# jgsimard/RustRobotics

Hardware: AMD Instinct MI355X
Metric: GN iterations/s (higher is better)
Workload: dtype f64; 1 GPU; intel (1728 poses / 4830 edges / dim 5184), Gauss-Newton, one graph on one GPU; solver=GaussNewton, parallelism=single

## Files before the change

### rustrobotics_amd/csrc/kernels.hip.h

```cpp
#pragma once
#include <hip/hip_runtime.h>

#include <cstdint>
#include <type_traits>

#ifndef RRPGO_CHAIN_PRIO
#define RRPGO_CHAIN_PRIO 3
#endif

namespace rrpgo {

constexpr unsigned X_PENDING_WORD = 0x7ff8deadu;

template <typename T> struct VecT;
template <> struct VecT<float> { using V4 = float4; using V2 = float2; };
template <> struct VecT<double> { using V4 = double4; using V2 = double2; };

#ifndef RRPGO_LIN_GROUP
#define RRPGO_LIN_GROUP 8
#endif
constexpr int LIN_GROUP = RRPGO_LIN_GROUP;
constexpr int LIN_THREADS = 256;
constexpr int UPD_THREADS = 256;

// ... 1424 lines not shown
__device__ __forceinline__ void diag16_factor_invert_full(T *P, int M, int k0, int *err, T *wscr) {
  const int lane = threadIdx.x & 63, ll = lane & 31, q = lane & 15;
  const bool rowlane = ll < 16;
  const T *src = rowlane ? P + k0 * M + k0 + q : wscr + 16 * 17 + q;
  const int sstride = rowlane ? M : 16;
  T x[16];
#pragma unroll
  for (int c = 0; c < 16; c++) x[c] = src[c * sstride];
  const bool bad = chol16_dpp2<T>(x);
  if (bad && lane == 0) atomicOr(err, DEVERR_NOT_SPD);
  T *dst = rowlane ? P + k0 * M + k0 + q : wscr + q * 17;
  const int dstride = rowlane ? M : 1;
#pragma unroll
  for (int c = 0; c < 16; c++) dst[c * dstride] = x[c];
}
template <typename T>
__device__ __forceinline__ void diag16_factor_invert_part(T *P, int M, int k0, int nb, int *err, T *wscr) {
  const int lane = threadIdx.x & 63, ll = lane & 31, q = lane & 15;
  const bool rowlane = ll < 16;
  const bool prow = rowlane && q < nb;
  T *ident = wscr + 16 * 17;
  const T *src = prow ? P + k0 * M + k0 + q : ident + q;
  const int sstride = prow ? M : 16;
  T x[16];
#pragma unroll
  for (int c = 0; c < 16; c++) {
    const T *pc = (prow && c >= nb) ? ident + 1 : src + c * sstride;
    x[c] = *pc;
  }
  const bool bad = chol16_dpp2<T>(x, nb);
  if (bad && lane == 0) atomicOr(err, DEVERR_NOT_SPD);
  T *dump = wscr + 16;
  T *dst = prow ? P + k0 * M + k0 + q : rowlane ? dump : wscr + q * 17;
  const int dstride = prow ? M : rowlane ? 0 : 1;
#pragma unroll
  for (int c = 0; c < 16; c++) {
    T *pc = (prow && c >= nb) ? dump : dst + c * dstride;
    *pc = x[c];
  }
}
template <typename T> __device__ __forceinline__ void copy_w16(const T *wscr, T *wout) {
  const int lane = threadIdx.x & 63;
#pragma unroll
  for (int u = 0; u < 4; u++) {
    const int e = lane + 64 * u;
    wout[e] = wscr[(e & 15) * 17 + (e >> 4)];
  }
}
template <typename T> __device__ __forceinline__ void init_w16_identity(T *wscr, int tid, int nthreads) {
  for (int t = tid; t < 256; t += nthreads) wscr[16 * 17 + t] = (t >> 4) == (t & 15) ? (T)1 : (T)0;
}

struct NoUAddr { __device__ float *operator()(int, int) const { return nullptr; } };
template <typename T, int THREADS, bool FAST = false, typename UAddr = NoUAddr>
__device__ __forceinline__ void panel_factor(T *P, int M, int nc, int *err, T *wscr , T *wout,
                             unsigned long long *acc = nullptr, int nu = 0, UAddr uaddr = UAddr(), bool defer_u = false) {
  using MM = Mfma16<T>;
  constexpr int NB = 16;
  constexpr int NW = THREADS / 64;
  const int tid = threadIdx.x;
  const int wave = wave_index(), lane = tid & 63, li = lane & 15, lk = lane >> 4;
  RRPGO_ACC_DECL();
  int pend_k0 = -1;
  auto rest_update = [&](int pk0, int first_wave, int nwaves) {
    const int js = pk0 + NB;
    const int nj = (nc - js + 15) >> 4, ni = (M - js + 15) >> 4;
    int total = 0;
    for (int jb = 1; jb < nj; jb++) total += max(ni - jb, 0);
    const int nt = (nu + 15) >> 4;
    const int utotal = defer_u ? 0 : nt * (nt + 1) / 2;
    for (int t = wave - first_wave; t < total + utotal; t += nwaves) {
      if (t < total) {
        int jb = 1, rem = t;
        while (rem >= ni - jb) { rem -= ni - jb; jb++; }
        const int ib = jb + rem;
        tile_rank_update<T>(P, M, js + 16 * ib, js + 16 * jb, M, nc, pk0, pk0 + NB,
                            [&](int i, int j) { return P + j * M + i; });
      } else {
        if constexpr (!std::is_same<UAddr, NoUAddr>::value) {
          int jb = 0, rem = t - total;
          while (rem >= nt - jb) { rem -= nt - jb; jb++; }
          const int ib = jb + rem;
          tile_rank_update<T>(P + nc, M, 16 * ib, 16 * jb, nu, nu, pk0, pk0 + NB, uaddr);
        }
      }
    }
  };
  for (int k0 = 0; k0 < nc; k0 += NB) {
    const int nb = min(NB, nc - k0);
    RRPGO_ACC_BEGIN();
    constexpr bool fast = FAST;
    auto diag = [&] {
      static_assert(FAST, "the general diagonal-block form (fronts factored in place in global memory by this routine) was retired in r05");
      if (nb == NB) diag16_factor_invert_full<T>(P, M, k0, err, wscr);
      else diag16_factor_invert_part<T>(P, M, k0, nb, err, wscr);
    };
    if (NW == 1) {
      if (pend_k0 >= 0) rest_update(pend_k0, 0, 1);
      diag();
    } else if (wave == 0) {
      diag();
    } else if (pend_k0 >= 0) {
      rest_update(pend_k0, 1, NW - 1);
    }
    pend_k0 = -1;
    __syncthreads();
    RRPGO_ACC_END(acc, 7);
    RRPGO_ACC_BEGIN();
    {
      const int r0 = k0 + nb;
      const int ntiles = (M - r0 + 15) >> 4;
      T wa[4];
#pragma unroll
      for (int s4 = 0; s4 < 4; s4++) wa[s4] = wscr[(4 * s4 + lk) * 17 + li];
      if (fast && wout && wave == NW - 1) copy_w16<T>(wscr, wout + (k0 >> 4) * 256);
      for (int ib = wave; ib < ntiles; ib += NW) {
        const int i = r0 + 16 * ib + li;
        const T *arow = P + min(i, M - 1);
        typename MM::Acc x = {0, 0, 0, 0};
        T av[4];
#pragma unroll
        for (int s4 = 0; s4 < 4; s4++) av[s4] = arow[(k0 + min(4 * s4 + lk, nb - 1)) * M];
#pragma unroll
        for (int s4 = 0; s4 < 4; s4++) av[s4] = pin(av[s4]);
#pragma unroll
        for (int s4 = 0; s4 < 4; s4++) {
          const int j = 4 * s4 + lk;
          x = MM::mma(wa[s4], j < nb ? av[s4] : (T)0, x);
        }
#pragma unroll
        for (int r = 0; r < 4; r++) {
          const int c = MM::row(lane, r);
          if (i < M && c < nb) P[(k0 + c) * M + i] = x[r];
        }
      }
    }
    __syncthreads();
    RRPGO_ACC_END(acc, 8);
    const int js = k0 + nb;
    if (js < nc) {
      RRPGO_ACC_BEGIN();
      const int ni = (M - js + 15) >> 4;
      for (int ib = wave; ib < ni; ib += NW)
        tile_rank_update<T>(P, M, js + 16 * ib, js, M, nc, k0, k0 + nb,
                            [&](int i, int j) { return P + j * M + i; });
      RRPGO_ACC_END(acc, 9);
      if (js + NB < nc || nu > 0) pend_k0 = k0;
    }
  }
}


__device__ __forceinline__ void lds_barrier() { asm volatile("s_waitcnt lgkmcnt(0)\n\ts_barrier" ::: "memory"); }

template <typename T, int THREADS, bool IN_PLACE, bool FLOW = false>
__device__ void process_front(const FactorArgs<T> &a, int s, const SnMeta &m, T *P, T *U, int uld, T *dinv) {
  static_assert(!(FLOW && IN_PLACE), "the dataflow form is for fronts in LDS");
  const int tid = threadIdx.x;
  const int nc = m.nc, nr = m.nr;
  const int M = nc + nr + 1, nu = nr + 1;
  const int psize = M * nc, usize = nu * (nu + 1) / 2;
  RRPGO_STAMP(a, s, 0);
#ifdef RRPGO_STAMPS
  if (FLOW && tid == 0 && a.stamps) a.stamps[(int64_t)s * 12 + 10] = 0;
#endif
  constexpr int APRE = 2;
  const int32_t *asrc = a.fasm_src + m.asm_begin, *adst = a.fasm_dst + m.asm_begin;
  int pd[APRE];
  T pv[APRE], pb = 0;
#pragma unroll
  for (int u = 0; u < APRE; u++) {
    const int t = tid + u * THREADS;
    pd[u] = -1;
    pv[u] = 0;
    if (t < m.asm_count) { pd[u] = adst[t]; pv[u] = a.hvals[asrc[t]]; }
  }
  if (tid < nc) pb = a.b[a.perm[m.col0 + tid]];
  ChildMeta cnext{};
  int dnext = -1;
  if (m.child_count > 0) {
    cnext = a.child_meta[m.child_begin];
    if (FLOW) dnext = a.child_dep[m.child_begin];
  }
  if (IN_PLACE) {
    for (int64_t t = tid; t < (int64_t)M * M; t += THREADS) P[t] = 0;
  } else {
    if constexpr (sizeof(T) == 4) {
      using V4z = typename VecT<T>::V4;
      const int n4 = (psize + usize) >> 2;
      V4z *P4 = reinterpret_cast<V4z *>(P);
      for (int t = tid; t < n4; t += THREADS) P4[t] = V4z{0, 0, 0, 0};
      if (tid < ((psize + usize) & 3)) P[4 * n4 + tid] = 0;
    } else {
      for (int t = tid; t < psize + usize; t += THREADS) P[t] = 0;
    }
  }
  constexpr int EPRE = 4;
  int ed[EPRE];
  T ev[EPRE];
  auto child_u = [&](const ChildMeta &c) { return (c.uld > 0 ? a.lvals : c.uld < 0 ? a.xch : a.uvals) + c.uoff; };
  auto uc_ld = [&](const T *Uc, const Sc1Buf<T> &ub, int t) -> T {
    if constexpr (FLOW) return ub.ld((uint32_t)t * (uint32_t)sizeof(T));
    else return Uc[t];
  };
  auto prefetch_map = [&](const ChildMeta &c) {
#pragma unroll
    for (int u = 0; u < EPRE; u++) { ed[u] = -1; ev[u] = 0; }
    if (IN_PLACE || c.scat_ptr < 0) return;
// ... 54 lines not shown
#ifdef RRPGO_STAMPS
      if (tid == 0 && a.stamps) a.stamps[(int64_t)s * 12 + 10] += wall_clock64() - w0_;
#endif
    }
    __syncthreads();
    if (!IN_PLACE && c.scat_ptr >= 0) {
      const int32_t *map = a.scat + c.scat_ptr;
      const int cnt = c.ncu * (c.ncu + 1) / 2;
      [[maybe_unused]] const Sc1Buf<T> ub(Uc, FLOW ? (uint32_t)cnt * (uint32_t)sizeof(T) : 0u);
      if (FLOW && dep >= 0) prefetch_val(c);
#pragma unroll
      for (int u = 0; u < EPRE; u++)
        if (ed[u] >= 0) P[ed[u]] += ev[u];
      if (q + 1 < m.child_count) prefetch(cnext, dnext);
      int t = tid + EPRE * THREADS;
      for (; t + 3 * THREADS < cnt; t += 4 * THREADS) {
        const int d0 = map[t], d1 = map[t + THREADS], d2 = map[t + 2 * THREADS], d3 = map[t + 3 * THREADS];
        const T v0 = uc_ld(Uc, ub, t), v1 = uc_ld(Uc, ub, t + THREADS), v2 = uc_ld(Uc, ub, t + 2 * THREADS), v3 = uc_ld(Uc, ub, t + 3 * THREADS);
        if (d0 >= 0) P[d0] += v0;
        if (d1 >= 0) P[d1] += v1;
        if (d2 >= 0) P[d2] += v2;
        if (d3 >= 0) P[d3] += v3;
      }
      for (; t < cnt; t += THREADS) {
        const int d0 = map[t];
        if (d0 >= 0) P[d0] += uc_ld(Uc, ub, t);
      }
    } else {
      if (q + 1 < m.child_count) prefetch(cnext, dnext);
      const int32_t *rel = a.rel + c.rel_ptr;
      const int ncu = c.ncu;
      for (int t = tid; t < ncu * ncu; t += THREADS) {
        const int j = t / ncu, i = t - j * ncu;
        if (i < j || t == ncu * ncu - 1) continue;
        const T v = Uc[tri_index(ncu, c.uld, i, j)];
        const int li = rel[i], lj = rel[j];
        if (lj < nc) P[(int64_t)lj * M + li] += v;
        else U[tri_index(nu, uld, li - nc, lj - nc)] += v;
      }
    }
  }
  __syncthreads();
  RRPGO_STAMP(a, s, 3);
#ifndef RRPGO_DEFER_U_MIN
#define RRPGO_DEFER_U_MIN 128
#endif
  const bool defer_u = sizeof(T) == 4 && nu >= RRPGO_DEFER_U_MIN && nc > 16;
  auto uaddr = [&](int i, int j) {
    return IN_PLACE ? U + ((int64_t)j * uld + i) : U + (j * nu - ((j * (j - 1)) >> 1) + (i - j));
  };
  {
#ifdef RRPGO_STAMPS
  if (tid == 0 && a.stamps) { a.stamps[(int64_t)s * 12 + 7] = 0; a.stamps[(int64_t)s * 12 + 8] = 0; a.stamps[(int64_t)s * 12 + 9] = 0; }
  panel_factor<T, THREADS, !IN_PLACE>(P, M, nc, a.err, dinv, a.winv + (int64_t)m.wblk * 256, a.stamps ? a.stamps + (int64_t)s * 12 : nullptr, nu, uaddr, defer_u);
#else
  panel_factor<T, THREADS, !IN_PLACE>(P, M, nc, a.err, dinv, a.winv + (int64_t)m.wblk * 256, nullptr, nu, uaddr, defer_u);
#endif
  }
  RRPGO_STAMP(a, s, 4);
  {
    const int klast = defer_u ? 0 : ((nc - 1) >> 4) << 4;
    const int nt = (nu + 15) >> 4;
    const int wave = wave_index();
    [[maybe_unused]] T *Ug0 = (m.uld < 0 ? a.xch : a.uvals) + m.uoff;
    [[maybe_unused]] const Sc1Buf<T> ub0(Ug0, (FLOW && !IN_PLACE) ? (uint32_t)usize * (uint32_t)sizeof(T) : 0u);
    auto to_memory = [&](T *p, T v) { ub0.st((uint32_t)(p - U) * (uint32_t)sizeof(T), v); };
    for (int t = wave; t < nt * (nt + 1) / 2; t += THREADS / 64) {
      int jb = 0, rem = t;
      while (rem >= nt - jb) { rem -= nt - jb; jb++; }
      const int ib = jb + rem;
      if constexpr (FLOW && !IN_PLACE) tile_rank_update<T>(P + nc, M, 16 * ib, 16 * jb, nu, nu, klast, nc, uaddr, to_memory);
      else tile_rank_update<T>(P + nc, M, 16 * ib, 16 * jb, nu, nu, klast, nc, uaddr);
    }
  }
  if constexpr (FLOW && !IN_PLACE) dep_drain();
  __syncthreads();
  RRPGO_STAMP(a, s, 5);
  if (!IN_PLACE) {
    using V2 = typename VecT<T>::V2;
    T *Lg = a.lvals + m.loff;
    T *Ug = (m.uld < 0 ? a.xch : a.uvals) + m.uoff;
    if constexpr (FLOW) {
      (void)Ug;
      if (tid == 0) dep_flag_set(a.dep_flags + s);
      RRPGO_STAMP(a, s, 11);
    }
    if ((psize & 1) == 0) {
      const V2 *sp = reinterpret_cast<const V2 *>(P);
      V2 *dp = reinterpret_cast<V2 *>(Lg);
      for (int t = tid; t < (psize >> 1); t += THREADS) dp[t] = sp[t];
    } else {
      for (int t = tid; t < psize; t += THREADS) Lg[t] = P[t];
    }
    if constexpr (!FLOW)
      for (int t = tid; t < usize; t += THREADS) Ug[t] = U[t];
    __syncthreads();
  }
  RRPGO_STAMP(a, s, 6);
}

template <typename T, int THREADS>
__device__ void kform_front(const FactorArgs<T> &a, const SnMeta &m, T *P) {
  using MM = Mfma16<T>;
  constexpr int NW = THREADS / 64;
  const int nc = m.nc, M = nc + m.nr + 1;
  const int lane = threadIdx.x & 63, li = lane & 15;
  const int wave = wave_index();
  const int nblk = (nc + 15) >> 4, ntr = (M - nc + 15) >> 4;
  const T *Wg = a.winv + (int64_t)m.wblk * 256;
// ... 30 lines not shown
    }
  }
  for (int b = nblk - 1; b >= 1; b--) {
    lds_barrier();
    const int c0 = 16 * b, cw = min(16, nc - c0);
    w_load(b - 1, wq);
    for (int t = wave; t < ntr * b; t += NW) {
      const int bb = b - 1 - t / ntr, ib = t % ntr;
      const int j0 = 16 * bb;
      const int r = nc + 16 * ib + li, rc = min(r, M - 1);
      typename MM::Acc acc;
      T av[4], bv[4];
#pragma unroll
      for (int q = 0; q < 4; q++) acc[q] = P[(j0 + MM::row(lane, q)) * M + rc];
#pragma unroll
      for (int s = 0; s < 4; s++) {
        const int k = MM::row(lane, s), kc = min(k, cw - 1);
        av[s] = P[(j0 + li) * M + c0 + kc];
        bv[s] = P[(c0 + kc) * M + rc];
      }
#pragma unroll
      for (int s = 0; s < 4; s++) acc = MM::mma(MM::row(lane, s) < cw ? -av[s] : (T)0, bv[s], acc);
      if (bb == b - 1) {
        T bq[4];
#pragma unroll
        for (int q = 0; q < 4; q++) bq[q] = acc[q];
        w_tile(bb, ib, bq, wq);
      } else if (r < M) {
#pragma unroll
        for (int q = 0; q < 4; q++) P[(j0 + MM::row(lane, q)) * M + r] = acc[q];
      }
    }
  }
}

template <typename T, int THREADS>
__device__ void kform_task(const FactorArgs<T> &a, int sn_begin, int sn_end, T *P) {
  for (int si = sn_end - 1; si >= sn_begin; si--) {
    const SnMeta m = a.sn_meta[a.task_sn[si]];
    if (m.nr == 0) continue;
    if (si == sn_end - 1) {
      kform_front<T, THREADS>(a, m, P);
      continue;
    }
    const int psize = (m.nc + m.nr + 1) * m.nc;
    const T *Lg = a.lvals + m.loff;
    __syncthreads();
    for (int t = threadIdx.x; t < psize; t += THREADS) P[t] = mem_ld<true>(Lg + t);
    __syncthreads();
    kform_front<T, THREADS>(a, m, P);
  }
}

template <typename T, int THREADS>
__global__ void __launch_bounds__(THREADS) k_factor_tasks(FactorArgs<T> a) {
  if (opt_stopped(a.err)) return;
  extern __shared__ __align__(16) unsigned char smem_raw[];
  __shared__ T dinv[W16_SCR];
  T *smem = reinterpret_cast<T *>(smem_raw);
  init_w16_identity<T>(dinv, threadIdx.x, THREADS);
  if (THREADS > 256 && wave_index() == 0) __builtin_amdgcn_s_setprio(RRPGO_CHAIN_PRIO);
  const int task = a.task_begin + blockIdx.x;
  const int sbeg = a.task_ptr[task], send = a.task_ptr[task + 1];
  int snext = a.task_sn[sbeg];
  SnMeta mnext = a.sn_meta[snext];
  for (int si = sbeg; si < send; si++) {
    const int s = snext;
    const SnMeta m = mnext;
    if (si + 1 < send) {
      snext = a.task_sn[si + 1];
      mnext = a.sn_meta[snext];
    }
    process_front<T, THREADS, false>(a, s, m, smem, smem + (m.nc + m.nr + 1) * m.nc, 0, dinv);
  }
  if (a.kvals) kform_task<T, THREADS>(a, sbeg, send, smem);
}

#ifndef RRPGO_BIG_NB
#define RRPGO_BIG_NB 32
#endif
#ifndef RRPGO_BIG_SUPER
#define RRPGO_BIG_SUPER 128
#endif
constexpr int BIG_NB = RRPGO_BIG_NB;
constexpr int BIG_SUPER = RRPGO_BIG_SUPER;

__device__ __host__ __forceinline__ int big_schur_origin(int nc, int tile) {
  return nc <= BIG_SUPER ? nc : ((nc + tile - 1) & ~(tile - 1));
}
__device__ __host__ __forceinline__ int big_built_cols(int nc, int M) {
  const int r = ((nc + 127) / 128) * 128;
  return nc <= BIG_SUPER ? nc : (r < M ? r : M);
}

template <typename T> __global__ void __launch_bounds__(256) k_big_assemble(FactorArgs<T> a, int add) {
  if (opt_stopped(a.err)) return;
  const SnMeta m = a.task_meta[a.task_begin + blockIdx.y];
  T *F = a.lvals + m.loff;
  const int M = m.nc + m.nr + 1;
  const int gid = blockIdx.x * 256 + threadIdx.x, gsz = gridDim.x * 256;
  const int32_t *src = a.fasm_src + m.asm_begin, *dst = a.fasm_dst + m.asm_begin;
  if (add) {
    for (int t = gid; t < m.asm_count; t += gsz) F[dst[t]] += a.hvals[src[t]];
    for (int j = gid; j < m.nc; j += gsz) F[(int64_t)j * M + (M - 1)] += a.b[a.perm[m.col0 + j]];
  } else {
    for (int t = gid; t < m.asm_count; t += gsz) F[dst[t]] = a.hvals[src[t]];
    for (int j = gid; j < m.nc; j += gsz) F[(int64_t)j * M + (M - 1)] = a.b[a.perm[m.col0 + j]];
  }
}

template <typename T, int QB, bool SC1 = false, typename Args = FactorArgs<T>>
__device__ __forceinline__ void big_build_column(const Args &a, const ChildMeta *cm, int nkids, int M, int J, T *col, int lane) {
  for (int r0 = (J & ~63) + lane; r0 < M; r0 += 256) {
    T acc[4] = {0, 0, 0, 0};
    for (int q0 = 0; q0 < nkids; q0 += QB) {
      int jq[QB], last[QB], iq[QB][4];
      const T *ucol[QB];
#pragma unroll
      for (int qq = 0; qq < QB; qq++) {
        const ChildMeta c = cm[min(q0 + qq, nkids - 1)];
        const int32_t *inv = a.scat + c.scat_ptr;
        const int j = __builtin_amdgcn_readfirstlane(inv[J]);
        jq[qq] = q0 + qq < nkids ? j : -1;
        const int jc = max(jq[qq], 0);
        const T *Uc = (c.uld > 0 ? a.lvals : c.uld < 0 ? a.xch : a.uvals) + c.uoff;
        ucol[qq] = Uc + (c.uld > 0 ? (int64_t)jc * c.uld : (int64_t)jc * c.ncu - (int64_t)jc * (jc - 1) / 2 - jc);
// ... 1594 lines not shown
```

### rustrobotics_amd/csrc/lds_flow.hip.h

```cpp
#pragma once

namespace rrpgo {

struct alignas(128) LdsFlowTask {
  SnMeta m;
  int32_t sn;
  int32_t sn_begin, sn_end;
  int32_t kind;
  int32_t slices;
  int32_t bx, by;
  int32_t n_units;
  int32_t pad[8];
};
static_assert(sizeof(LdsFlowTask) == 128, "LdsFlowTask is one 128-byte line");

__device__ __forceinline__ int lds_flow_ticket(unsigned *ticket, int *slot) {
  if (threadIdx.x == 0) *slot = (int)atomicAdd(ticket, 1u);
  __syncthreads();
  return __builtin_amdgcn_readfirstlane(*slot);
}

template <typename T, int THREADS>
__global__ void __launch_bounds__(THREADS) k_factor_flow(FactorArgs<T> a, const LdsFlowTask *tasks, int n_tasks, unsigned *ticket) {
  extern __shared__ __align__(16) unsigned char smem_raw[];
  __shared__ T dinv[W16_SCR];
  __shared__ int ticket_slot[2];
  T *smem = reinterpret_cast<T *>(smem_raw);
  const bool stopped = opt_stopped(a.err);
  init_w16_identity<T>(dinv, threadIdx.x, THREADS);
  if (THREADS > 256 && wave_index() == 0) __builtin_amdgcn_s_setprio(RRPGO_CHAIN_PRIO);
  for (int round = 0;; round++) {
    const int tk = lds_flow_ticket(ticket, &ticket_slot[round & 1]);
    if (tk >= n_tasks || stopped) break;
    const LdsFlowTask tr = tasks[tk];
    int snext = tr.sn;
    SnMeta mnext = tr.m;
    for (int si = tr.sn_begin; si < tr.sn_end; si++) {
      const int s = snext;
      const SnMeta m = mnext;
      if (si + 1 < tr.sn_end) {
        snext = a.task_sn[si + 1];
        mnext = a.sn_meta[snext];
      }
      process_front<T, THREADS, false, true>(a, s, m, smem, smem + (m.nc + m.nr + 1) * m.nc, 0, dinv);
    }
    if (a.kvals) kform_task<T, THREADS>(a, tr.sn_begin, tr.sn_end, smem);
  }
}

__device__ __forceinline__ bool dep_wait_count(const unsigned *p, unsigned need, int *err, unsigned long long max_ticks) {
  bool ok = true;
  if (dep_flag_ld(p) < need) {
    const unsigned long long t0 = wall_clock64();
    for (unsigned spins = 1;; spins++) {
      __builtin_amdgcn_s_sleep(1);
      if (dep_flag_ld(p) >= need) break;
      if ((spins & 31u) == 0u) {
        const int e = __hip_atomic_load(err, __ATOMIC_RELAXED, __HIP_MEMORY_SCOPE_AGENT);
        if (e != 0 || wall_clock64() - t0 > max_ticks) {
          if (e == 0 && (threadIdx.x & 63) == 0) atomicOr(err, DEVERR_FLOW_TIMEOUT);
          ok = false;
          break;
        }
      }
    }
  }
  __builtin_amdgcn_fence(__ATOMIC_ACQUIRE, "wavefront");
  return ok;
}

template <typename T, int THREADS>
__global__ void __launch_bounds__(THREADS) k_solve_flow(FactorArgs<T> a, const LdsFlowTask *tasks, int n_tasks, unsigned *ticket, T *part, int64_t N) {
  extern __shared__ __align__(16) unsigned char smem_raw[];
  __shared__ int ticket_slot[2];
  T *smem = reinterpret_cast<T *>(smem_raw);
  const bool stopped = opt_stopped(a.err);
  for (int round = 0;; round++) {
    const int tk = lds_flow_ticket(ticket, &ticket_slot[round & 1]);
    if (tk >= n_tasks || stopped) break;
    const LdsFlowTask tr = tasks[tk];
    if (tr.kind == 1) {
      big_gemv_unit<T, true>(a, tr.m, part, N, tr.slices, tr.bx, tr.by, smem);
      dep_drain();
      __syncthreads();
      if (threadIdx.x == 0) __hip_atomic_fetch_add(a.dep_flags + a.parent_dep_self + tr.sn, 1u, __ATOMIC_RELAXED, __HIP_MEMORY_SCOPE_AGENT);
      continue;
    }
    if (tr.kind == 2) {
      dep_wait_count(a.dep_flags + a.parent_dep_self + tr.sn, (unsigned)tr.n_units, a.err, a.wait_ticks);
      solve_big_front<T, THREADS, true>(a, tr.m, smem, part, N, tr.slices);
      continue;
    }
    int snext = tr.sn;
    SnMeta mnext = tr.m;
    for (int si = tr.sn_end - 1; si >= tr.sn_begin; si--) {
      const int s = snext;
      const SnMeta m = mnext;
// ... 19 lines not shown
```

### rustrobotics_amd/csrc/pgo_api.hip

```cpp
#include <mutex>
#include <queue>
#include <hip/hip_runtime.h>

#include <algorithm>
#include <chrono>
#include <cmath>
#include <cstdio>
#include <cstdlib>
#include <cstring>
#include <functional>
#include <memory>
#include <stdexcept>
#include <string>
#include <thread>
#include <vector>

#include "../../include/rr_pgo.h"
#include "host_graph.h"
#include "kernels.hip.h"
#include "flow.hip.h"
#include "lds_flow.hip.h"
#include "selinv.hip.h"
#include "treesolve.hip.h"
#include "symbolic.h"
// ... 293 lines not shown
    int64_t ticket_word = 0;
    int wfill_begin = 0, wfill_end = 0;
    double est_us = 0;
  };
  std::vector<std::unique_ptr<FlowLevel>> flow_levels_;
  std::vector<SnMeta> host_task_meta_;
  std::vector<SnMeta> host_sn_meta_;
  DevBuf<int64_t> flow_wfill_;
  DevBuf<unsigned> flow_flags_;
  int flow_max_nf_ = 1 << 20;
  int flow_max_tasks_ = 1 << 20;
  bool xl_ = false;
  int xl_max_fronts_ = 256;
  int xl_level_tasks_ = 1 << 20;
  bool xl_refused_ = false;
  DevBuf<FlowRec> xl_recs_;
  std::vector<FlowRec> xl_host_;
  DevBuf<int2> xl_child_done_;
  DevBuf<unsigned long long> xl_trace_;
  int64_t xl_ticket_word_ = 0;
  static constexpr bool fused_assembly_ = true;
  static constexpr bool flow_deep_ = true;
  bool flow_exact_ = false;
  struct SolveFlowLevel { DevBuf<SolveFlowFront> fronts; DevBuf<SolveFlowTask> tasks; int n_tasks = 0; int64_t ticket_word = 0; };
  std::vector<std::unique_ptr<SolveFlowLevel>> solve_flow_;
  bool solve_flow_on_ = true;
  int flow_schur_min_ = 512;
  int flow_grid_ = 0;
  bool lds_flow_ = false;
  DevBuf<int32_t> child_dep_, parent_dep_;
  std::vector<int32_t> host_child_dep_;
  DevBuf<unsigned> dep_flags_;
  DevBuf<LdsFlowTask> lds_ftasks_, lds_stasks_;
  int lds_n_tasks_ = 0, lds_flow_cus_ = 256;
  std::vector<LdsFlowTask> host_stasks_;
  int lds_n_stasks_ = 0;
  std::vector<char> mid_in_flow_;
  unsigned long long wait_ticks_ = 200000000ull;
  int withheld_child_ = -1, withheld_parent_ = -1, withheld_level_ = -1, withheld_task_ = -1;
  int32_t withheld_parent_val_ = -1;
  FlowRec withheld_rec_{};
  static constexpr int kDeadFlagWords = 4096;
  bool gauge_ok_ = false;
  bool gauge_now_ = false;
  int gauge_root_ = -1;
  DevBuf<int32_t> gauge_col_node_;
  DevBuf<T> gauge_v_;
  double gauge_ox_ = 0, gauge_oy_ = 0, gauge_mu_t_ = 0, gauge_mu_r_ = 0;
  DevBuf<int64_t> pack_list_;
  int n_pack_ = 0, pack_max_nu_ = 0;
  DevBuf<T> hvals_, b_, x_, dx_ref_, lvals_, uvals_, winv_, xnew_, gemv_part_;
  DevBuf<T> kvals_;
  bool kform_ = false;
  double kform_bytes_ = 0, kform_flops_ = 0;
  DevBuf<T> svals_;
  DevBuf<SelMeta> sel_meta_;
  DevBuf<int32_t> sel_order_;
  std::vector<int32_t> sel_level_ptr_, sel_col_sn_;
  std::vector<int64_t> sel_soff_;
  size_t sel_lds_ = 0;
  bool sel_ready_ = false;
  EventHolder sel_ev_[4];
  double sel_ms_[3] = {0, 0, 0};
  DevBuf<TsMeta> ts_meta_;
  std::vector<int32_t> ts_depth_, ts_col_sn_;
  size_t ts_lds_ = 0;
  bool ts_ready_ = false;
  DevBuf<TsTask> ts_tasks_;
  DevBuf<int32_t> ts_child_, ts_unit_, ts_czrow_;
  DevBuf<CovQuery> ts_query_;
  DevBuf<T> ts_z_, ts_u_;
  DevBuf<double> ts_out_;
  EventHolder ts_ev_[4];
  double ts_ms_[3] = {0, 0, 0};
  static constexpr int kGemvSlices = 16;
  DevBuf<double> chi_partial_, norm_partial_, hist_;
  DevBuf<int> counter_, err_, blocks_done_;
  DevBuf<unsigned long long> stamps_;
  DevBuf<int32_t> task_ptr_, task_sn_, fasm_src_, fasm_dst_, fasm_colptr_, fdup_src_, fdup_dst_, scat_, rel_, perm_, sn_rows_;
  DevBuf<SnMeta> sn_meta_, task_meta_;
  DevBuf<ChildMeta> child_meta_;
  std::vector<int> step_solve_lds_;
  PinnedBuf<double> host_pair_;
  PinnedBuf<V4> state_stage_;
  EventHolder state_stage_ev_;
  std::vector<double> state_in_;
  DevBuf<V4> pose_saved_;
  OptSlot *opt_ring_ = nullptr;
  DevBuf<OptCtrl> opt_ctrl_;
  bool opt_active_ = false;
  bool opt_first_ = false;
  bool opt_lambda_dev_ = false;
  int opt_publish_ = 0;
  double opt_lambda0_ = 0.01;
  bool stop_dirty_ = false;
  bool sync_optimize_ = false;
  int n_lin_blocks_ = 0, n_upd_blocks_ = 0;
  bool no_graph_ = false, force_graph_ = false;
  bool edge_lin_ = false;
  bool edge_lin_wave_ = false;
  bool edge_lin_env_ = false, edge_lin_wave_env_ = false;
  int lin_blocks_pull_ = 0, lin_blocks_edge_ = 0;
  int robust_kind_ = ROBUST_NONE;
  double robust_delta_ = 1.0;
  DevBuf<uint8_t> robust_mask_;
  int host_counter_ = 0;
// ... 197 lines not shown
        m.nr = sym.sn_nrows[f];
        m.col0 = sym.sn_col0[f];
        m.uld = sym.sn_uld[f];
        m.asm_begin = (int32_t)sym.fasm_ptr[f];
        m.asm_count = (int32_t)(sym.fasm_ptr[f + 1] - sym.fasm_ptr[f]);
        m.dup_begin = (int32_t)sym.fdup_ptr[f];
        m.dup_count = (int32_t)(sym.fdup_ptr[f + 1] - sym.fdup_ptr[f]);
        m.child_begin = sym.child_ptr[f];
        m.child_count = sym.child_ptr[f + 1] - sym.child_ptr[f];
        if (sym.sn_rows_ptr[f] > 0x7fffffffLL) throw ApiError(RR_PGO_EUNSUPPORTED, "row structure exceeds 32-bit indexing");
        m.rows_ptr = (int32_t)sym.sn_rows_ptr[f];
        m.wblk = (int32_t)wblk_total;
        wblk_total += sym.sn_big[f] ? 4 * ((sym.sn_ncols[f] + 31) / 32) : (sym.sn_ncols[f] + 15) / 16;
        m.loff = sym.sn_loff[f];
        m.uoff = sym.sn_uoff[f];
        if (sym.sn_xch_off[f] >= 0 && !sym.sn_big[f]) {
          m.uld = -1;
          m.uoff = sym.sn_xch_off[f];
        }
      }
      for (size_t q = 0; q < cm.size(); q++) {
        const int c = sym.child_list[q];
        cm[q].uoff = sym.sn_uoff[c];
        cm[q].scat_ptr = sym.scat_ptr[c];
        cm[q].rel_ptr = sym.rel_ptr[c];
        cm[q].ncu = sym.sn_nrows[c] + 1;
        cm[q].uld = sym.sn_uld[c];
        if (sym.sn_xch_off[c] >= 0) {
          cm[q].uld = -1;
          cm[q].uoff = sym.sn_xch_off[c];
        }
      }
      sn_meta_.upload(meta);
      host_sn_meta_ = meta;
      {
        std::vector<SnMeta> tm(sym.task_ptr.size() - 1);
        for (size_t t = 0; t + 1 < sym.task_ptr.size(); t++) tm[t] = meta[sym.task_sn[sym.task_ptr[t]]];
        task_meta_.upload(tm);
        host_task_meta_ = tm;
        for (const Step &st : sym.steps)
          if (st.kind == STEP_BIG)
            for (int t = st.task_begin; t < st.task_end; t++) {
              const int sn = sym.task_sn[sym.task_ptr[t]];
              const int64_t Mf = sym.sn_ncols[sn] + sym.sn_nrows[sn] + 1;
              if (Mf * Mf * (int64_t)sizeof(T) >= (1LL << 32))
                throw ApiError(RR_PGO_EUNSUPPORTED, "a front of more than 4 GiB exceeds the 32-bit addressing of the big-front kernels");
            }
      }
      if (wblk_total > 0x7fffff00LL) throw ApiError(RR_PGO_EUNSUPPORTED, "too many diagonal blocks");
      winv_.alloc((size_t)wblk_total * 256 + 4);
      winv_.zero();
      kform_ = sym.flow_eligible && !sharded_ && world_ <= 1;
      if (const char *e = getenv("RR_PGO_SOLVE_KFORM")) kform_ = kform_ && std::atoi(e) != 0;
      if (kform_) {
        int64_t kend = 0;
        for (int f = 0; f < sym.S; f++)
          if (!sym.sn_big[f] && sym.sn_nrows[f] > 0) {
            const double nc = sym.sn_ncols[f], nu = sym.sn_nrows[f] + 1;
            kend = std::max<int64_t>(kend, sym.sn_loff[f] + (int64_t)(nc + nu) * sym.sn_ncols[f]);
            kform_bytes_ += (nc * (nc + 1) / 2 + 2 * nu * nc) * sizeof(T);
            kform_flops_ += nu * nc * nc;
          }
        kvals_.alloc((size_t)kend + 4);
        kvals_.zero();
      }
      {
        bool any_big = false;
        for (const Step &st : sym.steps) any_big = any_big || st.kind == STEP_BIG;
        xnew_.alloc(any_big ? (size_t)wblk_total * 256 + 4 : 4);
        xnew_.zero();
      }
      child_meta_.upload(cm);
      if (const char *e = getenv("RR_PGO_FLOW_TIMEOUT_MS")) wait_ticks_ = (unsigned long long)std::max(1.0, std::atof(e) * 1e5);
      if (sym.lds_flow) {
        if (sharded_ || world_ > 1) throw ApiError(RR_PGO_EUNSUPPORTED, "internal: dataflow schedule on a sharded handle");
        lds_flow_ = true;
        if (sym.steps.empty() || sym.steps[0].kind != STEP_TASKS || sym.steps[0].task_begin != 0)
          throw ApiError(RR_PGO_EUNSUPPORTED, "internal: the dataflow step must come first");
        for (size_t si = 1; si < sym.steps.size(); si++)
          if (sym.steps[si].kind != STEP_BIG) throw ApiError(RR_PGO_EUNSUPPORTED, "internal: a second LDS step behind the dataflow step");
        const int nt = sym.steps[0].task_end;
        std::vector<int32_t> task_of(sym.S, -1);
        for (size_t t = 0; t + 1 < sym.task_ptr.size(); t++)
          for (int q = sym.task_ptr[t]; q < sym.task_ptr[t + 1]; q++) task_of[sym.task_sn[q]] = (int)t;
        host_child_dep_.assign(cm.size(), -1);
        std::vector<int32_t> pdep(sym.S, -1);
        for (int f = 0; f < sym.S; f++) {
          for (int q = sym.child_ptr[f]; q < sym.child_ptr[f + 1]; q++) {
            const int c = sym.child_list[q];
            if (task_of[c] != task_of[f]) host_child_dep_[q] = c;
            else if (c > f) throw ApiError(RR_PGO_EUNSUPPORTED, "internal: child after its parent in one task");
          }
          const int pf = sym.sn_parent[f];
          if (pf >= 0 && !sym.sn_big[pf] && task_of[pf] != task_of[f]) pdep[f] = sym.S + pf;
        }
        child_dep_.upload(host_child_dep_);
        parent_dep_.upload(pdep);
        dep_flags_.alloc((size_t)2 * sym.S + 128);
        dep_flags_.zero();
        std::vector<LdsFlowTask> ft(nt), stk(nt);
        for (int t = 0; t < nt; t++) {
          LdsFlowTask r{};
          r.sn_begin = sym.task_ptr[t];
          r.sn_end = sym.task_ptr[t + 1];
          r.sn = sym.task_sn[r.sn_begin];
          r.m = meta[r.sn];
// ... 570 lines not shown

  void setup_gauge() {
    if (sizeof(T) != 4 || is3d_ || g_.anchor_node < 0 || sym_.S == 0) return;
    if (const char *e = getenv("RR_PGO_GAUGE")) if (std::atoi(e) == 0) return;
    const int root = sym_.S - 1;
    if (!sym_.sn_big[root] || !sym_.sn_huge[root] || sym_.sn_nrows[root] != 0) return;
    std::vector<int32_t> cn;
    double sx = 0, sy = 0, ext = 0;
    int n_se2 = 0, n_nodes = 0;
    for (int p = sym_.sn_first_pos[root]; p < sym_.sn_first_pos[root] + sym_.sn_npos[root]; p++) {
      const int node = sym_.order[p];
      const double *st = &g_.node_state[g_.node_state_off[node]];
      sx += st[0]; sy += st[1]; n_nodes++;
      n_se2 += g_.node_kind[node] == NODE_SE2;
      for (int t = 0; t < node_dim(g_.node_kind[node]); t++) cn.push_back((node << 2) | t);
    }
    if (n_se2 == 0 || (int)cn.size() != sym_.sn_ncols[root]) return;
    gauge_ox_ = sx / n_nodes; gauge_oy_ = sy / n_nodes;
    for (int p = sym_.sn_first_pos[root]; p < sym_.sn_first_pos[root] + sym_.sn_npos[root]; p++) {
      const double *st = &g_.node_state[g_.node_state_off[sym_.order[p]]];
      ext = std::max(ext, std::max(std::fabs(st[0] - gauge_ox_), std::fabs(st[1] - gauge_oy_)));
    }
    double w = 0;
    for (int k = 0; k < g_.n_edges(); k++) {
      const double *wi = &g_.edge_info[g_.edge_info_off[k]];
      w = std::max(w, std::fabs(wi[0]));
    }
    gauge_mu_t_ = w;
    gauge_mu_r_ = w / std::max(1.0, ext * ext);
    gauge_root_ = root;
    gauge_col_node_.upload(cn);
    gauge_v_.alloc(3 * cn.size());
    gauge_ok_ = true;
  }
  void launch_gauge_term() {
    GaugeArgs<T, S> ga;
    ga.pose = pose_.p;
    ga.col_node = gauge_col_node_.p;
    ga.nc = sym_.sn_ncols[gauge_root_];
    ga.M = ga.nc + sym_.sn_nrows[gauge_root_] + 1;
    ga.F = lvals_.p + sym_.sn_loff[gauge_root_];
    ga.v = gauge_v_.p;
    ga.ox = (S)gauge_ox_; ga.oy = (S)gauge_oy_;
    ga.mu_t = (T)gauge_mu_t_; ga.mu_r = (T)gauge_mu_r_;
    hipLaunchKernelGGL((k_gauge_vectors<T, S>), dim3((ga.nc + 255) / 256), dim3(256), 0, stream_, ga);
    hipLaunchKernelGGL((k_big_gauge<T, S>), dim3(ga.nc), dim3(256), 0, stream_, ga);
    check_launch("k_big_gauge");
  }

  static constexpr int kMaxLds = 160 * 1024 - 9216;

  template <int TH> void set_lds_attr() {
    HIPCHK(hipFuncSetAttribute((const void *)k_factor_tasks<T, TH>, hipFuncAttributeMaxDynamicSharedMemorySize, kMaxLds));
    HIPCHK(hipFuncSetAttribute((const void *)k_solve_tasks<T, TH>, hipFuncAttributeMaxDynamicSharedMemorySize, kMaxLds));
  }
  int level_max_nc(const Step &st) const {
    int max_nc = 1;
    for (int t = st.task_begin; t < st.task_end; t++) max_nc = std::max(max_nc, sym_.sn_ncols[sym_.task_sn[sym_.task_ptr[t]]]);
    return max_nc;
  }
  int gemv_slices(const Step &st) const {
    const int nf = st.task_end - st.task_begin, cb = (level_max_nc(st) + 63) / 64;
    int max_nr = 1;
    for (int t = st.task_begin; t < st.task_end; t++) max_nr = std::max(max_nr, sym_.sn_nrows[sym_.task_sn[sym_.task_ptr[t]]]);
    return std::max(1, std::min(std::min(kGemvSlices, (max_nr + 127) / 128), (768 + nf * cb - 1) / (nf * cb)));
  }
  void plan_mid_solve_tasks() {
    mid_in_flow_.assign(sym_.steps.size(), 0);
    if (!lds_flow_) return;
    bool on = true;
    if (const char *e = getenv("RR_PGO_SOLVE_MID_FLOW")) on = std::atoi(e) != 0;
    int top = (int)sym_.steps.size() - 1;
    while (on && top >= 1 && level_max_nc(sym_.steps[top]) >= sp_solve_min_nc_) top--;
    std::vector<LdsFlowTask> mid;
    int need = 1024;
    for (int i = top; on && i >= 1; i--) {
      const Step &st = sym_.steps[i];
      if (level_max_nc(st) >= sp_solve_min_nc_) { on = false; break; }
      const int R = gemv_slices(st);
      for (int pass = 1; pass <= 2; pass++)
        for (int t = st.task_begin; t < st.task_end; t++) {
          LdsFlowTask r{};
          r.sn_begin = sym_.task_ptr[t];
          r.sn_end = r.sn_begin + 1;
          r.sn = sym_.task_sn[r.sn_begin];
          r.m = host_sn_meta_[r.sn];
          r.kind = pass;
          r.slices = R;
          const int nc = sym_.sn_ncols[r.sn], nr = sym_.sn_nrows[r.sn];
          const int units = nr > 0 ? (nc + 63) / 64 * R : 0;
          if (pass == 2) {
            r.n_units = units;
            mid.push_back(r);
            need = std::max(need, ((nc + 3) & ~3) + 2 * 32 * 33 + 64);
          } else {
            for (int u = 0; u < units; u++) { r.bx = u / R; r.by = u % R; mid.push_back(r); }
          }
        }
    }
    if (on && !mid.empty() && (size_t)need * sizeof(T) <= (size_t)kMaxLds) {
      for (int i = top; i >= 1; i--) mid_in_flow_[i] = 1;
      step_solve_lds_[0] = std::max(step_solve_lds_[0], need);
      mid.insert(mid.end(), host_stasks_.begin(), host_stasks_.end());
      host_stasks_.swap(mid);
    }
    lds_n_stasks_ = (int)host_stasks_.size();
    lds_stasks_.upload(host_stasks_);
  }

  void configure_kernels() {
    set_lds_attr<64>();
    set_lds_attr<128>();
    set_lds_attr<256>();
    set_lds_attr<512>();
    HIPCHK(hipFuncSetAttribute((const void *)k_factor_tasks<T, 1024>, hipFuncAttributeMaxDynamicSharedMemorySize, kMaxLds));
    HIPCHK(hipFuncSetAttribute((const void *)k_solve_mid<T, 1024>, hipFuncAttributeMaxDynamicSharedMemorySize, kMaxLds));
    HIPCHK(hipFuncSetAttribute((const void *)k_factor_flow<T, 256>, hipFuncAttributeMaxDynamicSharedMemorySize, kMaxLds));
    HIPCHK(hipFuncSetAttribute((const void *)k_factor_flow<T, 512>, hipFuncAttributeMaxDynamicSharedMemorySize, kMaxLds));
    HIPCHK(hipFuncSetAttribute((const void *)k_factor_flow<T, 1024>, hipFuncAttributeMaxDynamicSharedMemorySize, kMaxLds));
    HIPCHK(hipFuncSetAttribute((const void *)k_solve_flow<T, 256>, hipFuncAttributeMaxDynamicSharedMemorySize, kMaxLds));
    HIPCHK(hipFuncSetAttribute((const void *)k_solve_flow<T, 512>, hipFuncAttributeMaxDynamicSharedMemorySize, kMaxLds));
  }

  template <int TH> void launch_factor_tasks(int nt, size_t lds, const FactorArgs<T> &a) {
    hipLaunchKernelGGL((k_factor_tasks<T, TH>), dim3(nt), dim3(TH), lds, stream_, a);
  }
  template <int TH> void launch_solve_tasks(int nt, size_t lds, const FactorArgs<T> &a) {
    hipLaunchKernelGGL((k_solve_tasks<T, TH>), dim3(nt), dim3(TH), lds, stream_, a);
  }

  LinArgs<T, S> lin_args(double lambda, int lm, int write_system, bool reference_prior = false) {
    if (write_system) gauge_now_ = gauge_ok_ && !lm && !reference_prior;
    LinArgs<T, S> a;
    a.n_nodes = n_list_;
    a.node_list = node_list_.p;
    a.pose = pose_.p;
    a.e_rec = e_rec_.p;
    a.e_idx = e_idx_.p;
    a.e_meas = e_meas_.p;
    a.e_info_a = e_info_a_.p;
    a.e_info_b = e_info_b_.p;
    a.e_slot = e_slot_.p;
    a.inc_ptr = inc_ptr_.p;
    a.inc_list = inc_list_.p;
    a.node_dim = node_dim_.p;
    a.node_offset = node_offset_.p;
    a.diag_off = diag_off_.p;
    a.hvals = hvals_.p;
    a.b = b_.p;
    a.chi2_partial = chi_partial_.p;
    a.anchor = (write_system && gauge_now_) ? -1 : g_.anchor_node;
    a.lambda = lm ? (S)lambda : (S)0;
    a.write_system = write_system;
    a.adds_diag = norm_counts_.p;
    a.zero_words = lds_flow_ ? dep_flags_.p : nullptr;
    a.n_zero_words = lds_flow_ ? 2 * sym_.S + 64 : 0;
    a.fill_words = lds_flow_ ? reinterpret_cast<unsigned *>(x_ptr_) : nullptr;
    a.n_fill_words = lds_flow_ ? (int)((size_t)g_.dim * sizeof(T) / 4) : 0;
    opt_lin_fields(a, lm);
    robust_fields(a);
    return a;
  }
  template <typename A> void robust_fields(A &a) const {
    a.robust_delta = (S)robust_delta_;
    a.robust_delta2 = (S)(robust_delta_ * robust_delta_);
    a.robust_mask = robust_mask_.n ? robust_mask_.p : nullptr;
  }
  template <typename A> void opt_lin_fields(A &a, int lm) {
    a.ctrl = opt_active_ ? opt_ctrl_.p : nullptr;
    a.err = err_.p;
    a.lambda_from_ctrl = (opt_active_ && opt_lambda_dev_ && lm) ? 1 : 0;
    a.reset_ctrl = (opt_active_ && opt_first_) ? 1 : 0;
    a.reset_lambda = opt_lambda0_;
    a.reset_tolerance = 1e-4;
    a.publish = opt_active_ ? opt_publish_ : 0;
    a.ring_host = opt_ring_;
    a.blocks_done = blocks_done_.p + 1;
    opt_first_ = false;
// ... 91 lines not shown
                           lin_args(lambda, lm, write_system, reference_prior));
    } else {
      LinArgs3<T, S> a;
      a.n_nodes = n_list_;
      a.node_list = node_list_.p;
      a.pose = pose_.p;
      a.e_idx = e_idx_.p;
      a.e_meas = e_meas_.p;
      a.e_info = e_info3_.p;
      a.e_slot = e_slot_.p;
      a.inc_ptr = inc_ptr_.p;
      a.inc_list = inc_list_.p;
      a.node_offset = node_offset_.p;
      a.diag_off = diag_off_.p;
      a.hvals = hvals_.p;
      a.b = b_.p;
      a.chi2_partial = chi_partial_.p;
      a.anchor = g_.anchor_node;
      a.lambda = lm ? (S)lambda : (S)0;
      a.write_system = write_system;
      a.adds_diag = norm_counts_.p;
      a.zero_words = lds_flow_ ? dep_flags_.p : nullptr;
      a.n_zero_words = lds_flow_ ? 2 * sym_.S + 64 : 0;
      a.fill_words = lds_flow_ ? reinterpret_cast<unsigned *>(x_ptr_) : nullptr;
      a.n_fill_words = lds_flow_ ? (int)((size_t)g_.dim * sizeof(T) / 4) : 0;
      opt_lin_fields(a, lm);
      robust_fields(a);
      if (robust_kind_ == ROBUST_HUBER) hipLaunchKernelGGL((k_linearize_se3<T, S, ROBUST_HUBER>), dim3(n_lin_blocks_), dim3(LIN_THREADS), 0, stream_, a);
      else if (robust_kind_ == ROBUST_CAUCHY) hipLaunchKernelGGL((k_linearize_se3<T, S, ROBUST_CAUCHY>), dim3(n_lin_blocks_), dim3(LIN_THREADS), 0, stream_, a);
      else hipLaunchKernelGGL((k_linearize_se3<T, S>), dim3(n_lin_blocks_), dim3(LIN_THREADS), 0, stream_, a);
    }
    check_launch("k_linearize");
    pend(RR_PGO_K_LINEARIZE);
  }

  void launch_factor() { launch_factor_range(0, sym_.steps.size()); }
  void launch_factor_range(size_t from, size_t to) {
    if (any_flow(from, to)) {
      int e0 = 0, e1 = 0;
      for (size_t si = from; si < to && si < flow_levels_.size(); si++)
        if (flow_levels_[si]) { if (e1 == 0) e0 = flow_levels_[si]->wfill_begin; e1 = flow_levels_[si]->wfill_end; }
      const int flag_wgs = (int)std::min<int64_t>(((int64_t)flow_flags_.n + 255) / 256, 256);
      hipLaunchKernelGGL(k_flow_reset<T>, dim3((unsigned)(flag_wgs + std::max(e1 - e0, 0))), dim3(256), 0, stream_, flow_flags_.p, (int64_t)flow_flags_.n, flag_wgs,
                         winv_.p, flow_wfill_.p + 2 * e0, xnew_.p);
      check_launch("k_flow_reset");
    }
    if (lds_flow_ && from == 0 && to > 0) {
      const Step &st = sym_.steps[0];
      pbegin();
      const size_t lds = (size_t)st.max_lds_elems * sizeof(T);
      const FactorArgs<T> a = factor_args(0);
      const int grid = std::min(lds_n_tasks_, lds_flow_cus_);
      unsigned *ticket = dep_flags_.p + 2 * sym_.S;
      if (std::min(st.threads, factor_threads_max_) <= 256)
        hipLaunchKernelGGL((k_factor_flow<T, 256>), dim3(grid), dim3(256), lds, stream_, a, (const LdsFlowTask *)lds_ftasks_.p, lds_n_tasks_, ticket);
      else if (std::min(st.threads, factor_threads_max_) <= 512)
        hipLaunchKernelGGL((k_factor_flow<T, 512>), dim3(grid), dim3(512), lds, stream_, a, (const LdsFlowTask *)lds_ftasks_.p, lds_n_tasks_, ticket);
      else
        hipLaunchKernelGGL((k_factor_flow<T, 1024>), dim3(grid), dim3(1024), lds, stream_, a, (const LdsFlowTask *)lds_ftasks_.p, lds_n_tasks_, ticket);
      check_launch("k_factor_flow");
      pend(RR_PGO_K_FACTOR);
      from = 1;
    }
    if (xl_ && from == 1 && to == sym_.steps.size()) {
      pbegin();
      launch_flow_xl();
      pend(RR_PGO_K_BIG_FLOW);
      return;
    }
    for (size_t si = from; si < to; si++) {
      const Step &st = sym_.steps[si];
      pbegin();
      if (st.kind == STEP_TASKS) {
        const int nt = st.task_end - st.task_begin;
        const size_t lds = (size_t)st.max_lds_elems * sizeof(T);
        FactorArgs<T> a = factor_args(st.task_begin);
        const int fth = step_threads(st, nt, factor_threads_max_);
        if (fth == 64) launch_factor_tasks<64>(nt, lds, a);
        else if (fth == 128) launch_factor_tasks<128>(nt, lds, a);
        else if (fth == 256) launch_factor_tasks<256>(nt, lds, a);
        else if (fth <= 512) launch_factor_tasks<512>(nt, lds, a);
        else launch_factor_tasks<1024>(nt, lds, a);
        pend(RR_PGO_K_FACTOR);
      } else {
        launch_big_level(st, true);
        pend(RR_PGO_K_BIGFRONT);
      }
    }
  }

  int step_threads(const Step &st, int, int cap) const { return std::min(st.threads, cap); }

  int launch_big_level(const Step &st, bool do_launch) {
    const FactorArgs<T> a = factor_args(st.task_begin);
    const int nf = st.task_end - st.task_begin;
    int maxM = 0, max_nc = 0, n = 0;
    int64_t max_asm = 0;
    bool any_dup = false;
    std::vector<int> fr(nf);
    for (int z = 0; z < nf; z++) {
      const int s = sym_.task_sn[sym_.task_ptr[st.task_begin + z]];
      fr[z] = s;
      maxM = std::max(maxM, sym_.sn_ncols[s] + sym_.sn_nrows[s] + 1);
      max_nc = std::max(max_nc, sym_.sn_ncols[s]);
      max_asm = std::max<int64_t>(max_asm, std::max<int64_t>(sym_.fasm_ptr[s + 1] - sym_.fasm_ptr[s], sym_.sn_ncols[s]));
      any_dup = any_dup || sym_.fdup_ptr[s + 1] > sym_.fdup_ptr[s];
    }
    auto rows_max = [&](int from) {
      int r = 0;
      for (int s : fr)
        if (sym_.sn_ncols[s] > from) r = std::max(r, sym_.sn_ncols[s] + sym_.sn_nrows[s] + 1 - from);
      return r;
// ... 1921 lines not shown
```

Measured before the change: 7578 GN iterations/s.

## Fuse panel triangular solve with trailing rank update in f64 panel factor

```diff
diff --git a/rustrobotics_amd/csrc/kernels.hip.h b/rustrobotics_amd/csrc/kernels.hip.h
--- a/rustrobotics_amd/csrc/kernels.hip.h
+++ b/rustrobotics_amd/csrc/kernels.hip.h
@@ -1500,7 +1500,7 @@
 }
 
 struct NoUAddr { __device__ float *operator()(int, int) const { return nullptr; } };
-template <typename T, int THREADS, bool FAST = false, typename UAddr = NoUAddr>
+template <typename T, int THREADS, bool FAST = false, bool FUSED = false, typename UAddr = NoUAddr>
 __device__ __forceinline__ void panel_factor(T *P, int M, int nc, int *err, T *wscr , T *wout,
                              unsigned long long *acc = nullptr, int nu = 0, UAddr uaddr = UAddr(), bool defer_u = false) {
   using MM = Mfma16<T>;
@@ -1543,11 +1543,30 @@
       if (nb == NB) diag16_factor_invert_full<T>(P, M, k0, err, wscr);
       else diag16_factor_invert_part<T>(P, M, k0, nb, err, wscr);
     };
+    constexpr bool fused_form = FUSED && sizeof(T) == 8 && NW > 1;
+    const bool fused_blk = fused_form && nb == NB && k0 + NB < nc;
     if (NW == 1) {
       if (pend_k0 >= 0) rest_update(pend_k0, 0, 1);
       diag();
     } else if (wave == 0) {
       diag();
+      if constexpr (fused_form) {
+        if (fused_blk) {
+          asm volatile("s_waitcnt lgkmcnt(0)" ::: "memory");
+          const int i = k0 + NB + li;
+          const T *arow = P + min(i, M - 1) + (k0 + lk) * M, *wop = wscr + lk * 17 + li;
+          T wa[4], av[4];
+#pragma unroll
+          for (int q = 0; q < 4; q++) { wa[q] = wop[q * 68]; av[q] = arow[q * 4 * M]; }
+          typename MM::Acc x = {0, 0, 0, 0};
+#pragma unroll
+          for (int q = 0; q < 4; q++) x = MM::mma(wa[q], av[q], x);
+          if (i < M) {
+#pragma unroll
+            for (int r = 0; r < 4; r++) P[(k0 + MM::row(lane, r)) * M + i] = x[r];
+          }
+        }
+      }
     } else if (pend_k0 >= 0) {
       rest_update(pend_k0, 1, NW - 1);
     }
@@ -1555,6 +1574,57 @@
     __syncthreads();
     RRPGO_ACC_END(acc, 7);
     RRPGO_ACC_BEGIN();
+    if constexpr (fused_form) {
+      if (fused_blk) {
+        const int js = k0 + NB;
+        const int ntiles = (M - js + 15) >> 4;
+        const T *wop = wscr + lk * 17 + li;
+        T wa[4];
+#pragma unroll
+        for (int q = 0; q < 4; q++) wa[q] = wop[q * 68];
+        if (fast && wout && wave == NW - 1) copy_w16<T>(wscr, wout + (k0 >> 4) * 256);
+        const T *x0p = P + min(js + li, nc - 1) + (k0 + lk) * M;
+        for (int ib = wave; ib < ntiles; ib += NW) {
+          const int i = js + 16 * ib + li, ic = min(i, M - 1);
+          const T *arow = P + ic + (k0 + lk) * M;
+          T *pc[4];
+          T av[4], xo[4];
+          typename MM::Acc a2;
+#pragma unroll
+          for (int r = 0; r < 4; r++) pc[r] = P + min(min(js + MM::row(lane, r), nc - 1), ic) * M + ic;
+#pragma unroll
+          for (int q = 0; q < 4; q++) av[q] = arow[q * 4 * M];
+#pragma unroll
+          for (int q = 0; q < 4; q++) xo[q] = x0p[q * 4 * M];
+#pragma unroll
+          for (int r = 0; r < 4; r++) a2[r] = -*pc[r];
+          typename MM::Acc x;
+          if (ib == 0) {
+#pragma unroll
+            for (int q = 0; q < 4; q++) x[q] = av[q];
+          } else {
+            x = typename MM::Acc{0, 0, 0, 0};
+#pragma unroll
+            for (int q = 0; q < 4; q++) x = MM::mma(wa[q], av[q], x);
+            if (i < M) {
+#pragma unroll
+              for (int r = 0; r < 4; r++) P[(k0 + MM::row(lane, r)) * M + i] = x[r];
+            }
+          }
+#pragma unroll
+          for (int q = 0; q < 4; q++) a2 = MM::mma(xo[q], x[q], a2);
+#pragma unroll
+          for (int r = 0; r < 4; r++) {
+            const int j = js + MM::row(lane, r);
+            if (i < M && j < nc && i >= j) *pc[r] = -a2[r];
+          }
+        }
+        __syncthreads();
+        RRPGO_ACC_END(acc, 9);
+        if (js + NB < nc || nu > 0) pend_k0 = k0;
+        continue;
+      }
+    }
     {
       const int r0 = k0 + nb;
       const int ntiles = (M - r0 + 15) >> 4;
@@ -1586,7 +1656,7 @@
     __syncthreads();
     RRPGO_ACC_END(acc, 8);
     const int js = k0 + nb;
-    if (js < nc) {
+    if (!fused_form && js < nc) {
       RRPGO_ACC_BEGIN();
       const int ni = (M - js + 15) >> 4;
       for (int ib = wave; ib < ni; ib += NW)
@@ -1601,7 +1671,7 @@
 
 __device__ __forceinline__ void lds_barrier() { asm volatile("s_waitcnt lgkmcnt(0)\n\ts_barrier" ::: "memory"); }
 
-template <typename T, int THREADS, bool IN_PLACE, bool FLOW = false>
+template <typename T, int THREADS, bool IN_PLACE, bool FLOW = false, bool FUSED = false>
 __device__ void process_front(const FactorArgs<T> &a, int s, const SnMeta &m, T *P, T *U, int uld, T *dinv) {
   static_assert(!(FLOW && IN_PLACE), "the dataflow form is for fronts in LDS");
   const int tid = threadIdx.x;
@@ -1762,9 +1832,9 @@
   {
 #ifdef RRPGO_STAMPS
   if (tid == 0 && a.stamps) { a.stamps[(int64_t)s * 12 + 7] = 0; a.stamps[(int64_t)s * 12 + 8] = 0; a.stamps[(int64_t)s * 12 + 9] = 0; }
-  panel_factor<T, THREADS, !IN_PLACE>(P, M, nc, a.err, dinv, a.winv + (int64_t)m.wblk * 256, a.stamps ? a.stamps + (int64_t)s * 12 : nullptr, nu, uaddr, defer_u);
+  panel_factor<T, THREADS, !IN_PLACE, FUSED>(P, M, nc, a.err, dinv, a.winv + (int64_t)m.wblk * 256, a.stamps ? a.stamps + (int64_t)s * 12 : nullptr, nu, uaddr, defer_u);
 #else
-  panel_factor<T, THREADS, !IN_PLACE>(P, M, nc, a.err, dinv, a.winv + (int64_t)m.wblk * 256, nullptr, nu, uaddr, defer_u);
+  panel_factor<T, THREADS, !IN_PLACE, FUSED>(P, M, nc, a.err, dinv, a.winv + (int64_t)m.wblk * 256, nullptr, nu, uaddr, defer_u);
 #endif
   }
   RRPGO_STAMP(a, s, 4);
@@ -1901,7 +1971,7 @@
   }
 }
 
-template <typename T, int THREADS>
+template <typename T, int THREADS, bool FUSED = false>
 __global__ void __launch_bounds__(THREADS) k_factor_tasks(FactorArgs<T> a) {
   if (opt_stopped(a.err)) return;
   extern __shared__ __align__(16) unsigned char smem_raw[];
@@ -1920,7 +1990,7 @@
       snext = a.task_sn[si + 1];
       mnext = a.sn_meta[snext];
     }
-    process_front<T, THREADS, false>(a, s, m, smem, smem + (m.nc + m.nr + 1) * m.nc, 0, dinv);
+    process_front<T, THREADS, false, false, FUSED>(a, s, m, smem, smem + (m.nc + m.nr + 1) * m.nc, 0, dinv);
   }
   if (a.kvals) kform_task<T, THREADS>(a, sbeg, send, smem);
 }
diff --git a/rustrobotics_amd/csrc/lds_flow.hip.h b/rustrobotics_amd/csrc/lds_flow.hip.h
--- a/rustrobotics_amd/csrc/lds_flow.hip.h
+++ b/rustrobotics_amd/csrc/lds_flow.hip.h
@@ -20,7 +20,7 @@
   return __builtin_amdgcn_readfirstlane(*slot);
 }
 
-template <typename T, int THREADS>
+template <typename T, int THREADS, bool FUSED = false>
 __global__ void __launch_bounds__(THREADS) k_factor_flow(FactorArgs<T> a, const LdsFlowTask *tasks, int n_tasks, unsigned *ticket) {
   extern __shared__ __align__(16) unsigned char smem_raw[];
   __shared__ T dinv[W16_SCR];
@@ -42,7 +42,7 @@
         snext = a.task_sn[si + 1];
         mnext = a.sn_meta[snext];
       }
-      process_front<T, THREADS, false, true>(a, s, m, smem, smem + (m.nc + m.nr + 1) * m.nc, 0, dinv);
+      process_front<T, THREADS, false, true, FUSED>(a, s, m, smem, smem + (m.nc + m.nr + 1) * m.nc, 0, dinv);
     }
     if (a.kvals) kform_task<T, THREADS>(a, tr.sn_begin, tr.sn_end, smem);
   }
diff --git a/rustrobotics_amd/csrc/pgo_api.hip b/rustrobotics_amd/csrc/pgo_api.hip
--- a/rustrobotics_amd/csrc/pgo_api.hip
+++ b/rustrobotics_amd/csrc/pgo_api.hip
@@ -369,6 +369,7 @@
   DevBuf<T> hvals_, b_, x_, dx_ref_, lvals_, uvals_, winv_, xnew_, gemv_part_;
   DevBuf<T> kvals_;
   bool kform_ = false;
+  bool panel_fused_ = sizeof(T) == 8;
   double kform_bytes_ = 0, kform_flops_ = 0;
   DevBuf<T> svals_;
   DevBuf<SelMeta> sel_meta_;
@@ -672,6 +673,7 @@
       winv_.zero();
       kform_ = sym.flow_eligible && !sharded_ && world_ <= 1;
       if (const char *e = getenv("RR_PGO_SOLVE_KFORM")) kform_ = kform_ && std::atoi(e) != 0;
+      if (const char *e = getenv("RR_PGO_PANEL_FUSED")) panel_fused_ = panel_fused_ && std::atoi(e) != 0;
       if (kform_) {
         int64_t kend = 0;
         for (int f = 0; f < sym.S; f++)
@@ -1348,6 +1350,8 @@
 
   template <int TH> void set_lds_attr() {
     HIPCHK(hipFuncSetAttribute((const void *)k_factor_tasks<T, TH>, hipFuncAttributeMaxDynamicSharedMemorySize, kMaxLds));
+    if constexpr (sizeof(T) == 8 && TH > 64)
+      HIPCHK(hipFuncSetAttribute((const void *)k_factor_tasks<T, TH, true>, hipFuncAttributeMaxDynamicSharedMemorySize, kMaxLds));
     HIPCHK(hipFuncSetAttribute((const void *)k_solve_tasks<T, TH>, hipFuncAttributeMaxDynamicSharedMemorySize, kMaxLds));
   }
   int level_max_nc(const Step &st) const {
@@ -1410,6 +1414,12 @@
     set_lds_attr<256>();
     set_lds_attr<512>();
     HIPCHK(hipFuncSetAttribute((const void *)k_factor_tasks<T, 1024>, hipFuncAttributeMaxDynamicSharedMemorySize, kMaxLds));
+    if constexpr (sizeof(T) == 8) {
+      HIPCHK(hipFuncSetAttribute((const void *)k_factor_tasks<T, 1024, true>, hipFuncAttributeMaxDynamicSharedMemorySize, kMaxLds));
+      HIPCHK(hipFuncSetAttribute((const void *)k_factor_flow<T, 256, true>, hipFuncAttributeMaxDynamicSharedMemorySize, kMaxLds));
+      HIPCHK(hipFuncSetAttribute((const void *)k_factor_flow<T, 512, true>, hipFuncAttributeMaxDynamicSharedMemorySize, kMaxLds));
+      HIPCHK(hipFuncSetAttribute((const void *)k_factor_flow<T, 1024, true>, hipFuncAttributeMaxDynamicSharedMemorySize, kMaxLds));
+    }
     HIPCHK(hipFuncSetAttribute((const void *)k_solve_mid<T, 1024>, hipFuncAttributeMaxDynamicSharedMemorySize, kMaxLds));
     HIPCHK(hipFuncSetAttribute((const void *)k_factor_flow<T, 256>, hipFuncAttributeMaxDynamicSharedMemorySize, kMaxLds));
     HIPCHK(hipFuncSetAttribute((const void *)k_factor_flow<T, 512>, hipFuncAttributeMaxDynamicSharedMemorySize, kMaxLds));
@@ -1419,7 +1429,22 @@
   }
 
   template <int TH> void launch_factor_tasks(int nt, size_t lds, const FactorArgs<T> &a) {
+    if constexpr (sizeof(T) == 8 && TH > 64) {
+      if (panel_fused_) {
+        hipLaunchKernelGGL((k_factor_tasks<T, TH, true>), dim3(nt), dim3(TH), lds, stream_, a);
+        return;
+      }
+    }
     hipLaunchKernelGGL((k_factor_tasks<T, TH>), dim3(nt), dim3(TH), lds, stream_, a);
+  }
+  template <int TH> void launch_factor_flow(int grid, size_t lds, const FactorArgs<T> &a, unsigned *ticket) {
+    if constexpr (sizeof(T) == 8) {
+      if (panel_fused_) {
+        hipLaunchKernelGGL((k_factor_flow<T, TH, true>), dim3(grid), dim3(TH), lds, stream_, a, (const LdsFlowTask *)lds_ftasks_.p, lds_n_tasks_, ticket);
+        return;
+      }
+    }
+    hipLaunchKernelGGL((k_factor_flow<T, TH>), dim3(grid), dim3(TH), lds, stream_, a, (const LdsFlowTask *)lds_ftasks_.p, lds_n_tasks_, ticket);
   }
   template <int TH> void launch_solve_tasks(int nt, size_t lds, const FactorArgs<T> &a) {
     hipLaunchKernelGGL((k_solve_tasks<T, TH>), dim3(nt), dim3(TH), lds, stream_, a);
@@ -1617,12 +1642,9 @@
       const FactorArgs<T> a = factor_args(0);
       const int grid = std::min(lds_n_tasks_, lds_flow_cus_);
       unsigned *ticket = dep_flags_.p + 2 * sym_.S;
-      if (std::min(st.threads, factor_threads_max_) <= 256)
-        hipLaunchKernelGGL((k_factor_flow<T, 256>), dim3(grid), dim3(256), lds, stream_, a, (const LdsFlowTask *)lds_ftasks_.p, lds_n_tasks_, ticket);
-      else if (std::min(st.threads, factor_threads_max_) <= 512)
-        hipLaunchKernelGGL((k_factor_flow<T, 512>), dim3(grid), dim3(512), lds, stream_, a, (const LdsFlowTask *)lds_ftasks_.p, lds_n_tasks_, ticket);
-      else
-        hipLaunchKernelGGL((k_factor_flow<T, 1024>), dim3(grid), dim3(1024), lds, stream_, a, (const LdsFlowTask *)lds_ftasks_.p, lds_n_tasks_, ticket);
+      if (std::min(st.threads, factor_threads_max_) <= 256) launch_factor_flow<256>(grid, lds, a, ticket);
+      else if (std::min(st.threads, factor_threads_max_) <= 512) launch_factor_flow<512>(grid, lds, a, ticket);
+      else launch_factor_flow<1024>(grid, lds, a, ticket);
       check_launch("k_factor_flow");
       pend(RR_PGO_K_FACTOR);
       from = 1;
```

Result: slower. 7381 GN iterations/s (-2.6%).
